# qiyunzhu/woltka

Hardware: AMD Instinct MI355X
Metric: alignment records/sec classified (higher is better)
Workload: dtype u8; 1 GPU; synthetic SAM text of 50M reads x <=16 hits (10.50 GB) resident in HBM, 2M-node taxonomy, ranks phylum,genus,species: device tokenizer per 64 MB block + one weighted histogram per sample (the kernels of `woltka classify`, host link left out); records_per_gpu=250034804, reads_per_gpu=50000000

## Files before the change

woltka_amd/csrc/wk_dtok_fused.hpp:

```cpp
#pragma once
#include "wk_dtok.hpp"
#include "wk_dtok_planes.hpp"

namespace wk {

constexpr uint32_t kFzThreads = 512;
constexpr uint32_t kFzWaves = kFzThreads / kWave;
constexpr uint32_t kFzTile = 16384;
constexpr uint32_t kFzBack = 1024;
constexpr uint32_t kFzFwd = 3072;
constexpr uint32_t kFzWin = kFzTile + kFzBack + kFzFwd;
constexpr uint32_t kFzChunks = kFzWin / 16 + 1;
constexpr uint32_t kFzChunksPerWave = (kFzChunks + kFzWaves - 1) / kFzWaves;
constexpr uint32_t kFzRounds = (kFzChunksPerWave + kWave - 1) / kWave;
constexpr uint32_t kFzLines = 1024;
constexpr uint32_t kFzStreams = 4;
constexpr uint32_t kFzCap = 1024;
static_assert(kFzCap >= kFzLines, "a window's records fit an empty buffer");
static_assert(kFzWin + 32 < 65536, "window offsets fit 16 bits");
constexpr uint32_t kFzCarry = 256;
static_assert(kFzCarry + kFzLines <= kFpMaxLines && kFzThreads % kWave == 0, "a window's owned lines fit the planes, a wave's lines one word");

constexpr uint32_t kDtokSpill = 64;

struct FusedArgs {
    const unsigned char* text;
    uint32_t n;
    uint32_t open_end;
    uint32_t span;
    const struct DictSlot8* dict8;
    const uint4* names16;
    uint32_t dict_mask;
    const unsigned char* arena;
    uint2* unknown;
    uint32_t unknown_cap;
    DtokState* state;
    DtokState* host_state;
    const unsigned long long* backup_prev;
    unsigned long long* backup_next;
    uint32_t* host_seq;
    uint32_t seq;
    StreamSet streams;
    const int32_t* submap;
    uint32_t n_submap;
    uint32_t ablate;
};

static_assert(sizeof(DtokState) % 8 == 0, "the packed totals are aligned");
__device__ __forceinline__ unsigned long long* fz_totals(DtokState* state) { return reinterpret_cast<unsigned long long*>(state + 1); }

__global__ void dtok_fused_begin_kernel(unsigned long long* __restrict__ backup, const unsigned long long* __restrict__ cursor, DtokState* state) {
    if (threadIdx.x < (uint32_t)kMaxStreams) backup[threadIdx.x] = cursor[threadIdx.x];
    if (threadIdx.x == 0) {
        *state = DtokState{0u, 0u, 0ull, 0ull, 0ull, 0u, 0u};
        *fz_totals(state) = 0ull;
    }
}

template <int kCtrl, int kRowMask>
__device__ __forceinline__ uint32_t fz_dpp_add(uint32_t v) {
    return v + (uint32_t)__builtin_amdgcn_update_dpp(0, (int)v, kCtrl, kRowMask, 0xF, false);
}
__device__ __forceinline__ uint32_t fz_wave_scan(uint32_t v) {
    static_assert(kWave == 64, "four rows of sixteen lanes");
    v = fz_dpp_add<0x111, 0xF>(v);
    v = fz_dpp_add<0x112, 0xF>(v);
    v = fz_dpp_add<0x114, 0xF>(v);
    v = fz_dpp_add<0x118, 0xF>(v);
    v = fz_dpp_add<0x142, 0xA>(v);
    v = fz_dpp_add<0x143, 0xC>(v);
    return v;
}
__device__ __forceinline__ uint32_t fz_last_lane(uint32_t v) { return (uint32_t)__builtin_amdgcn_readlane((int)v, kWave - 1); }
__device__ __forceinline__ uint32_t fz_wave_sum(uint32_t v) { return fz_last_lane(fz_wave_scan(v)); }
__device__ __forceinline__ unsigned long long fz_first_lane64(unsigned long long v) {
    return ((unsigned long long)(uint32_t)__builtin_amdgcn_readfirstlane((int)(uint32_t)(v >> 32)) << 32) |
           (uint32_t)__builtin_amdgcn_readfirstlane((int)(uint32_t)v);
}
constexpr uint32_t kFzNlBits = 11, kFzNlMask = (1u << kFzNlBits) - 1u;
static_assert(kFzRounds == 3 && kWave * 16u <= kFzNlMask, "two fields of 11 bits");
static_assert(kFzChunksPerWave > 2u * kWave && (kFzChunksPerWave - 2u * kWave) * 16u < (1u << (32u - 2u * kFzNlBits)), "and one of 10");

__device__ __forceinline__ uint4 fz_load_stream(const unsigned char* p) {
    typedef uint32_t u32x4 __attribute__((ext_vector_type(4)));
    const u32x4 v = __builtin_nontemporal_load(reinterpret_cast<const u32x4*>(p));
    return make_uint4(v.x, v.y, v.z, v.w);
}
__device__ __forceinline__ unsigned long long fz_load64(const unsigned char* p) {
    unsigned long long w;
    __builtin_memcpy(&w, p, 8);
    return w;
}
__device__ __forceinline__ uint32_t fz_load32(const unsigned char* p) {
    uint32_t w;
    __builtin_memcpy(&w, p, 4);
    return w;
}
__device__ __forceinline__ unsigned long long fz_eq_bytes(unsigned long long w, unsigned char c) {
    const unsigned long long x = w ^ (0x0101010101010101ull * c);
    return ~(((x & 0x7F7F7F7F7F7F7F7Full) + 0x7F7F7F7F7F7F7F7Full) | x | 0x7F7F7F7F7F7F7F7Full);
}
__device__ __forceinline__ uint32_t fz_marks32(uint32_t w, uint32_t c4) {
    const uint32_t x = w ^ c4;
    return ~(((x & 0x7F7F7F7Fu) + 0x7F7F7F7Fu) | x | 0x7F7F7F7Fu);
}
__device__ __forceinline__ unsigned long long fz_low_bytes(unsigned long long w, uint32_t k) {
    return k >= 8u ? w : (w & ((1ull << (8u * k)) - 1ull));
}

__device__ __forceinline__ unsigned long long fz_hash(const unsigned char* p, uint32_t n) {
    unsigned long long h = 0xcbf29ce484222325ull ^ ((unsigned long long)n * 0x9E3779B97F4A7C15ull);
    while (n >= 8u) {
        h = (h ^ fz_load64(p)) * 0x100000001b3ull;
        h ^= h >> 29;
        p += 8;
        n -= 8u;
    }
    const unsigned long long v = n ? fz_low_bytes(fz_load64(p), n) : 0ull;
    h = (h ^ v) * 0x100000001b3ull;
    h ^= h >> 32;
    h *= 0x9E3779B97F4A7C15ull;
    return h ^ (h >> 29);
}

__device__ __forceinline__ bool fz_same(const unsigned char* x, const unsigned char* y, uint32_t n) {
    while (n >= 8u) {
        if (fz_load64(x) != fz_load64(y)) return false;
        x += 8;
        y += 8;
        n -= 8u;
    }
    return n == 0u || fz_low_bytes(fz_load64(x) ^ fz_load64(y), n) == 0ull;
}

// ... 44 lines not shown
    while (pos > 0u) {
        const uint32_t e = pos - 1u;
        uint32_t s = e;
        while (s > 0u && text[s - 1u] != '\n') --s;
        uint32_t tab[3], nt = 0;
        for (uint32_t p = s; p < e && nt < 3u; ++p)
            if (text[p] == '\t') tab[nt++] = p;
        if (nt == 3u && !(tab[2] - tab[1] == 2u && text[tab[1] + 1u] == '*')) {
            if (tab[0] - s != qn) return true;
            for (uint32_t k = 0; k < qn; ++k)
                if (text[s + k] != q[k]) return true;
            return false;
        }
        pos = s;
    }
    return true;
}

constexpr uint32_t kFiSubj = (1u << 23) - 1u;
constexpr uint32_t kFiMateShift = 24;
constexpr uint32_t kFiMapped = 1u << 26;
constexpr uint32_t kFiStart = 1u << 27;
constexpr uint32_t kFiExcl = 1u << 29;
constexpr uint32_t kFiDropped = 1u << 30;
constexpr uint32_t kFiRead = kFiMapped | (3u << kFiMateShift);
constexpr uint32_t kFiKey = kFiRead | kFiSubj;
constexpr uint32_t kFzPad = 8;

__device__ __forceinline__ uint32_t fz_octet(uint32_t z_lo, uint32_t z_hi) { return (((z_lo >> 7) | (z_hi >> 3)) * 0x00204081u >> 21) & 255u; }

__device__ __forceinline__ uint32_t fz_newlines16(uint4 v) {
    return fz_octet(fz_marks32(v.x, 0x0A0A0A0Au), fz_marks32(v.y, 0x0A0A0A0Au)) | (fz_octet(fz_marks32(v.z, 0x0A0A0A0Au), fz_marks32(v.w, 0x0A0A0A0Au)) << 8);
}

__device__ __forceinline__ uint32_t fz_tabs32(const unsigned char* p) {
    unsigned long long w[4];
#pragma unroll
    for (uint32_t i = 0; i < 4; ++i) w[i] = fz_load64(p + 8u * i);
    uint32_t m = 0;
#pragma unroll
    for (uint32_t i = 0; i < 4; ++i)
        m |= fz_octet(fz_marks32((uint32_t)w[i], 0x09090909u), fz_marks32((uint32_t)(w[i] >> 32), 0x09090909u)) << (8u * i);
    return m;
}

__global__ void __launch_bounds__(kFzThreads) __attribute__((amdgpu_waves_per_eu(6, 6))) dtok_fused_kernel(FusedArgs a) {
    __shared__ __attribute__((aligned(16))) unsigned char txt[kFzChunks * 16 + 32];
    __shared__ uint16_t ls[kFzLines + 2];
    __shared__ uint16_t f_qn[kFzLines], f_rb[kFzLines], f_rn[kFzLines];
    __shared__ __attribute__((aligned(16))) uint32_t info_[kFzPad + kFzCarry + kFzLines + kFzPad + 8];
    __shared__ uint32_t carry[kFzCarry];
    __shared__ unsigned long long planes[kFpPlanes][kFpWords];
    __shared__ uint32_t rbuf[kFzStreams][kFzCap];
    __shared__ uint32_t rcnt[kFzStreams];
    __shared__ unsigned long long newc_packed;
    static_assert(kFzStreams <= 4 && kFzLines < 65536, "four 16-bit counts");
    __shared__ unsigned long long gbase[kFzStreams];
    __shared__ uint32_t wtot[kFzWaves];
    __shared__ unsigned long long gbase_out[kMaxStreams];
    __shared__ unsigned long long wg_totals;
    __shared__ uint32_t own[4];
    __shared__ uint32_t wg_flags;
    uint32_t* const info = info_ + kFzPad + kFzCarry;

    const uint32_t tid = threadIdx.x, lane = tid & (kWave - 1), wave = tid / kWave;
    const uint32_t n_streams = a.streams.n_streams;
    if (tid < kFzStreams) rcnt[tid] = 0u;
    if (tid == 0) newc_packed = 0ull;
    if (tid == 0) wg_flags = 0u;
    if (tid == 0) wg_totals = 0ull;
    uint32_t my_flags = 0, my_reads = 0, my_lines = 0;
    const uint32_t text_end = a.n + (a.open_end ? 1u : 0u);

    auto flush_all = [&](bool last) {
        __syncthreads();
        if (tid < n_streams) {
            const uint32_t cnt = (a.ablate & 64u) ? 0u : rcnt[tid];
            unsigned long long base = 0ull;
            if (cnt) {
                base = atomicAdd(&a.streams.cursor[tid], (unsigned long long)cnt);
                if (base + cnt > a.streams.cap) atomicOr(&wg_flags, kDtokSpill);
            }
            gbase[tid] = base;
        }
        __syncthreads();
        for (uint32_t k = 0; k < n_streams; ++k) {
            const uint32_t cnt = (a.ablate & 64u) ? 0u : rcnt[k];
            const unsigned long long base = gbase[k];
            for (uint32_t i = tid; i < cnt; i += kFzThreads)
                if (base + i < a.streams.cap) a.streams.out[k][base + i] = rbuf[k][i];
        }
        if (last) return;
        __syncthreads();
        if (tid < n_streams) rcnt[tid] = 0u;
        __syncthreads();
    };

    const uint32_t t0 = blockIdx.x * a.span;
    const uint32_t t1 = a.n - t0 > a.span ? t0 + a.span : a.n;
    const uint32_t span_w1 = (uint32_t)min((unsigned long long)t1 + kFzFwd, (unsigned long long)text_end);
    uint32_t wpos = t0 >= kFzBack ? t0 - kFzBack : 0u;
    uint32_t mode = 0u;
    uint32_t counted = t0;
    bool wide = false;
    uint32_t nc = 0u;
    uint32_t cq_pos = 0u, cq_len = 0u;
    const uint32_t max_trips = a.span / 16u + 2u;
    for (uint32_t trip = 0;; ++trip) {
        if (trip >= max_trips) {
            my_flags |= kDtokSpill;
            break;
        }
        const uint32_t w0 = wpos & ~15u;
        const uint32_t lead = wpos - w0;
        const uint32_t w1 = (uint32_t)min((mode == 0u ? (unsigned long long)t0 + kFzTile + kFzFwd : (unsigned long long)w0 + kFzWin),
                                           (unsigned long long)(wide ? text_end : span_w1));
        const bool to_end = w1 == text_end;
        const bool last_win = wide || w1 == span_w1;
        __syncthreads();
        if (tid < 3u) own[tid] = tid < 2u ? 0xFFFFFFFFu : 0u;
        if (tid < kFzPad) info[-(int32_t)nc - 1 - (int32_t)tid] = kFiStart;
        for (uint32_t i = tid; i < nc; i += kFzThreads) info[(int32_t)i - (int32_t)nc] = carry[i];

        uint4 v[kFzRounds];
#pragma unroll
        for (uint32_t r = 0; r < kFzRounds; ++r) {
            const uint32_t cw = r * kWave + lane;
            const uint32_t p = w0 + (wave * kFzChunksPerWave + cw) * 16u;
            v[r] = make_uint4(0u, 0u, 0u, 0u);
            if (cw < kFzChunksPerWave && p < a.n && p < w1) v[r] = fz_load_stream(a.text + p);
        }
        uint32_t marks[kFzRounds];
        uint32_t nl_packed = 0;
        const uint32_t in_lo = max(wpos, counted), in_hi = min(min(w1, a.n), t1);
        const uint32_t wave_c0 = (uint32_t)__builtin_amdgcn_readfirstlane((int)(wave * kFzChunksPerWave));
#pragma unroll
        for (uint32_t r = 0; r < kFzRounds; ++r) {
            const uint32_t cw = r * kWave + lane;
            const uint32_t c = wave * kFzChunksPerWave + cw;
            const uint32_t p = w0 + c * 16u;
            marks[r] = 0u;
            const uint32_t rc0 = wave_c0 + r * kWave, rp0 = w0 + rc0 * 16u;
            const bool interior = (r + 1u) * kWave <= kFzChunksPerWave && rc0 + kWave <= kFzChunks && rp0 >= in_lo &&
                                  (unsigned long long)rp0 + kWave * 16u <= in_hi;
            if (interior) {
                *reinterpret_cast<uint4*>(txt + c * 16u) = v[r];
                const uint32_t m = fz_newlines16(v[r]);
                const uint32_t cnt = (uint32_t)__popc(m);
                my_lines += cnt;
                marks[r] = m;
                nl_packed |= cnt << (kFzNlBits * r);
            } else if (cw < kFzChunksPerWave && c < kFzChunks) {
                *reinterpret_cast<uint4*>(txt + c * 16u) = v[r];
                if (p < w1) {
                    uint32_t m = fz_newlines16(v[r]);
                    if (p + 16u > a.n) m &= p >= a.n ? 0u : (1u << (a.n - p)) - 1u;
                    if (p >= counted && p < t1) my_lines += (uint32_t)__popc(m);
                    if (a.open_end && a.n >= p && a.n < p + 16u) m |= 1u << (a.n - p);
                    if (p + 16u > w1) m &= (1u << (w1 - p)) - 1u;
                    if (p < wpos) m &= ~((1u << (wpos - p)) - 1u);
                    marks[r] = m;
                    nl_packed |= (uint32_t)__popc(m) << (kFzNlBits * r);
                }
            }
        }
        const uint32_t nl_inc = fz_wave_scan(nl_packed);
        const uint32_t nl_wave = fz_last_lane(nl_inc);
        if (lane == 0) wtot[wave] = (nl_wave & kFzNlMask) + ((nl_wave >> kFzNlBits) & kFzNlMask) + (nl_wave >> (2u * kFzNlBits));
        __syncthreads();
        uint32_t before = 0, total_nl = 0;
#pragma unroll
        for (uint32_t w = 0; w < kFzWaves; ++w) {
            before += w < wave ? wtot[w] : 0u;
            total_nl += wtot[w];
        }
        const bool too_many = total_nl + 1u > kFzLines || (a.ablate & (32u | 512u));
        if (too_many) {
            if (!(a.ablate & 512u)) my_flags |= kDtokSpill;
        } else {
            if (tid == 0) ls[0] = (uint16_t)lead;
            uint32_t line = before;
#pragma unroll
            for (uint32_t r = 0; r < kFzRounds; ++r) {
                const uint32_t c = wave * kFzChunksPerWave + r * kWave + lane;
                uint32_t at = line + ((nl_inc >> (kFzNlBits * r)) & kFzNlMask) - (uint32_t)__popc(marks[r]);
                uint32_t m = marks[r];
                while (m) {
                    const uint32_t b = (uint32_t)__ffs((int)m) - 1u;
                    ls[++at] = (uint16_t)(c * 16u + b + 1u);
                    m &= m - 1u;
                }
                line += (nl_wave >> (kFzNlBits * r)) & kFzNlMask;
            }
        }
        __syncthreads();
        const uint32_t trail = too_many ? wpos : w0 + (uint32_t)__builtin_amdgcn_readfirstlane((int)(uint32_t)ls[total_nl]);
        if (!too_many && last_win && trail >= t0 && trail < t1) my_flags |= kDtokSpill;
        const uint32_t first_line = mode != 0u || w0 == 0u ? 0u : 1u;
        const uint32_t n_lines = too_many ? 0u : total_nl;
        if (tid == 0 && first_line) info[0] = 0u;

        for (uint32_t k = first_line + tid; k < n_lines; k += kFzThreads) {
            const uint32_t s = ls[k], e = (uint32_t)ls[k + 1] - 1u;
            uint32_t tab[3] = {0, 0, 0}, nt = 0;
            if (!(a.ablate & 256u)) {
                uint32_t m = fz_tabs32(txt + s);
                if (e - s < 32u) m &= (1u << (e - s)) - 1u;
                nt = min((uint32_t)__popc(m), 3u);
                tab[0] = s + (uint32_t)__ffs((int)m) - 1u;
                m &= m - 1u;
                tab[1] = s + (uint32_t)__ffs((int)m) - 1u;
                m &= m - 1u;
                tab[2] = s + (uint32_t)__ffs((int)m) - 1u;
                for (uint32_t p = s + 32u; nt < 3u && p < e; p += 32u) {
                    m = fz_tabs32(txt + p);
                    if (e - p < 32u) m &= (1u << (e - p)) - 1u;
                    for (; m && nt < 3u; m &= m - 1u) {
                        const uint32_t q = p + (uint32_t)__ffs((int)m) - 1u;
                        if (nt == 0u)
                            tab[0] = q;
                        else if (nt == 1u)
                            tab[1] = q;
                        else
                            tab[2] = q;
                        ++nt;
                    }
                }
            }
            uint32_t word = 0;
            if (a.ablate & 16u) {
            } else if (nt < 3u) {
                my_flags |= kDtokShortLine;
            } else {
                const uint32_t fl = tab[1] - tab[0] - 1u;
                const unsigned long long fw = fz_load64(txt + tab[0] + 1u);
                uint32_t flag = 0;
                bool digits = fl >= 1u && fl <= 6u;
                for (uint32_t i = 0; i < fl && i < 6u; ++i) {
                    const uint32_t d = ((uint32_t)(fw >> (8u * i)) & 0xFFu) - (uint32_t)'0';
                    digits &= d <= 9u;
                    flag = flag * 10u + d;
                }
                const uint32_t rb = tab[1] + 1u, rn = tab[2] - rb;
                if (!digits) {
                    my_flags |= kDtokShortLine;
                } else if (rn == 1u && txt[rb] == '*') {
                } else {
                    const uint32_t mate = (flag >> 6) & 3u;
                    if (mate == 3u) my_flags |= kDtokBothMates;
                    word = kFiMapped | (mate << kFiMateShift);
                    f_qn[k] = (uint16_t)(tab[0] - s);
                    f_rb[k] = (uint16_t)rb;
                    f_rn[k] = (uint16_t)rn;
                }
            }
            info[k] = word;
        }
        __syncthreads();

        for (uint32_t k = first_line + tid; k < n_lines; k += kFzThreads) {
            if (!(info[k] & kFiMapped) || w0 + ls[k] < t0) continue;
            const unsigned char* name = txt + f_rb[k];
            const uint32_t rn = f_rn[k];
            FzProbe probe;
            if (!(a.ablate & 1u)) probe = fz_probe_begin(a, name, rn);
            uint32_t j = k;
            bool found = false;
            while (j > first_line) {
                --j;
                if (info[j] & kFiMapped) {
                    found = true;
                    break;
                }
            }
            bool start;
            if (a.ablate & 8u)
                start = true;
            else if (found)
                start = f_qn[j] != f_qn[k] || !fz_same(txt + ls[k], txt + ls[j], f_qn[k]);
            else if (nc)
                start = f_qn[k] != cq_len || !fz_same(txt + ls[k], a.text + cq_pos, cq_len);
            else if (mode == 1u || wpos == 0u)
                start = true;
            else
                start = fz_starts_run_slow(a.text, w0 + ls[first_line], txt + ls[k], f_qn[k]);
            int32_t sid = (a.ablate & 1u) ? (int32_t)(fz_load32(name + 4) % 1000u) : fz_probe_end(a, probe, name, rn, w0 + f_rb[k]);
            bool excluded = false;
            if (a.submap && sid >= 0) {
                if ((uint32_t)sid < a.n_submap) {
                    sid = a.submap[sid];
                    if (sid == kLineExcluded) {
                        excluded = true;
                        sid = 0;
                    }
                } else {
                    my_flags |= kDtokSpill;
                    sid = -1;
                }
            }
            info[k] |= (start ? kFiStart : 0u) | (excluded ? kFiExcl : 0u) | (sid < 0 ? kFiSubj : ((uint32_t)sid & kFiSubj));
            if (start) {
                atomicMin(&own[w0 + ls[k] < t1 ? 0 : 1], k);
                atomicMax(&own[2], k);
            }
        }
        __syncthreads();
        const uint32_t o0 = (uint32_t)__builtin_amdgcn_readfirstlane((int)own[0]), o1 = (uint32_t)__builtin_amdgcn_readfirstlane((int)own[1]);
        const uint32_t last = (uint32_t)__builtin_amdgcn_readfirstlane((int)own[2]);
        const uint32_t lpos = w0 + (uint32_t)__builtin_amdgcn_readfirstlane((int)(uint32_t)ls[o0 != 0xFFFFFFFFu ? last : 0u]);
        const bool has_first = nc != 0u || o0 != 0xFFFFFFFFu;
        const int32_t first_own = nc ? -(int32_t)nc : (int32_t)o0;
        int32_t ka = 0, kb = 0;
        uint32_t next = 0u, next_mode = 0u, nc_next = 0u;
        bool more = false, again = false, put_aside = false;
        if (too_many) {
            if ((a.ablate & (32u | 512u)) && !last_win) {
                next = w1;
                next_mode = 2u;
                more = true;
            }
        } else if (o1 != 0xFFFFFFFFu) {
            kb = (int32_t)o1;
            ka = has_first ? first_own : kb;
        } else if (to_end) {
            kb = (int32_t)n_lines;
            ka = has_first ? first_own : kb;
        } else if (last_win && a.span <= kFzTile) {
            if (o0 != 0xFFFFFFFFu) my_flags |= kDtokSpill;
        } else if (o0 != 0xFFFFFFFFu && (nc != 0u || last != o0 || lpos > wpos)) {
            kb = (int32_t)last;
            ka = first_own;
            next = lpos;
            next_mode = 1u;
            more = true;
            again = last_win;
        } else if (o0 != 0xFFFFFFFFu && last_win && !wide) {
            next = wpos;
            next_mode = 1u;
            more = again = true;
        } else if (o0 != 0xFFFFFFFFu || nc != 0u) {
            put_aside = true;
        } else if (!last_win) {
            next = trail;
            next_mode = 2u;
            more = trail > wpos && trail < t1;
            if (trail <= wpos) my_flags |= kDtokSpill;
        }
        if (put_aside) {
            if (tid == 0) {
                uint32_t c = nc;
                for (uint32_t k = first_line; k < n_lines; ++k) {
                    const uint32_t w = info[k];
                    if (w & kFiMapped) {
                        if (c < kFzCarry) carry[c] = w & ~kFiDropped;
                        ++c;
                    }
                }
                own[3] = c;
            }
            __syncthreads();
            nc_next = (uint32_t)__builtin_amdgcn_readfirstlane((int)own[3]);
            if (nc_next > kFzCarry || trail <= wpos) {
                my_flags |= kDtokSpill;
                nc_next = 0u;
            } else {
                if (nc == 0u) {
                    cq_pos = wpos;
                    cq_len = (uint32_t)__builtin_amdgcn_readfirstlane((int)(uint32_t)f_qn[0]);
                }
                next = trail;
                next_mode = 2u;
                more = true;
                again = last_win;
            }
        }
        for (int32_t k0 = ka; k0 < kb; k0 += (int32_t)kFzThreads) {
            const int32_t k = k0 + (int32_t)tid;
            const uint32_t mk = k < kb ? info[k] : 0u;
            const bool mapped = (mk & kFiMapped) != 0u, excl = mapped && (mk & kFiExcl);
            if (excl) {
                int32_t j = k;
                while (!(info[j] & kFiStart)) --j;
                atomicOr(&info[j], kFiDropped);
            }
            bool dup = false;
            if (mapped && !excl && !(mk & kFiStart) && !(a.ablate & 2u)) {
                bool done = false;
                for (int32_t j = k; !done; j -= 8) {
                    uint32_t w[8];
#pragma unroll
                    for (uint32_t i = 0; i < 8; ++i) w[i] = info[j - 1 - (int32_t)i];
#pragma unroll
                    for (uint32_t i = 0; i < 8; ++i) {
                        dup |= !done && ((w[i] ^ mk) & kFiKey) == 0u;
                        done |= (w[i] & kFiStart) != 0u;
                    }
                }
            }
            const bool first = mapped && !excl && !dup;
            const uint32_t mate = (mk >> kFiMateShift) & 3u;
            const uint32_t wi = (uint32_t)__builtin_amdgcn_readfirstlane((int)((uint32_t)(k0 - ka) / kWave + wave));
            const bool put = lane == 0 && wi < kFpWords;
            const unsigned long long p_start = __ballot(mapped && (mk & kFiStart));
            if (put) planes[kFpStart][wi] = p_start;
#pragma unroll
            for (uint32_t m = 0; m < 4; ++m) {
                const unsigned long long p_first = __ballot(first && mate == m);
                if (put) planes[kFpFirst + m][wi] = p_first;
            }
        }
        __syncthreads();
        for (int32_t k0 = ka; k0 < kb; k0 += (int32_t)kFzThreads) {
            const int32_t k = k0 + (int32_t)tid;
            bool rec = false;
            uint32_t word = 0, sl = 0, at = 0;
            const uint32_t li = (uint32_t)(k - ka);
            const uint32_t mk = k < kb ? info[k] : 0u;
            const unsigned long long* const mine = planes[kFpFirst + ((mk >> kFiMateShift) & 3u)];
            if (k < kb && ((mine[li / 64u] >> (li % 64u)) & 1ull) && !(a.ablate & 4u)) {
                uint32_t pos = 0, size = 1;
                bool dropped = (mk & kFiStart) && (mk & kFiDropped);
                if (!(a.ablate & (2u | 128u))) {
                    const FpRead r = fp_read(planes[kFpStart], mine, li, (uint32_t)(kb - ka));
                    pos = r.pos;
                    size = r.size;
                    dropped = (info[ka + (int32_t)r.head] & kFiDropped) != 0u;
                }
                if (size > (uint32_t)WK_WEIGHT_MAX_K) my_flags |= kDtokBigRead;
                const uint32_t s = mk & kFiSubj;
                if (s != kFiSubj && !dropped) {
                    rec = true;
                    word = s | ((pos & 15u) << kWordSubjBits) | ((size & 31u) << kWordSizeShift);
                    sl = s / kSliceBins;
                    if (sl >= n_streams) sl = n_streams - 1u;
                    my_reads += pos == 0u ? 1u : 0u;
                }
            }
            {
                unsigned long long add = 0;
                uint32_t mine_before = 0;
                for (uint32_t s2 = 0; s2 < n_streams; ++s2) {
                    const unsigned long long m = __ballot(rec && sl == s2);
                    add |= (unsigned long long)__popcll(m) << (16u * s2);
                    if (rec && sl == s2) mine_before = (uint32_t)__popcll(m & ((1ull << lane) - 1ull));
                }
                if (add) {
                    unsigned long long base = 0;
                    if (lane == 0) base = atomicAdd(&newc_packed, add);
                    base = fz_first_lane64(base);
                    at = (uint32_t)(base >> (16u * sl)) & 0xFFFFu;
                    at += mine_before;
                }
            }
            __syncthreads();
            const unsigned long long newc = newc_packed;
            bool full = false;
            for (uint32_t s2 = 0; s2 < n_streams; ++s2) full |= rcnt[s2] + ((uint32_t)(newc >> (16u * s2)) & 0xFFFFu) > kFzCap;
            if (full) flush_all(false);
            if (rec) rbuf[sl][rcnt[sl] + at] = word;
            __syncthreads();
            if (tid < n_streams) rcnt[tid] += (uint32_t)(newc >> (16u * tid)) & 0xFFFFu;
            if (tid == 0) newc_packed = 0ull;
            __syncthreads();
        }
        if (!more) break;
        wpos = next;
        mode = next_mode;
        wide = again;
        nc = nc_next;
        counted = w1;
    }
    if (my_flags) atomicOr(&wg_flags, my_flags);
    {
        const uint32_t reads_w = fz_wave_sum(my_reads), lines_w = fz_wave_sum(my_lines);
        const unsigned long long t = ((unsigned long long)lines_w << 32) | reads_w;
        if (lane == 0 && t) atomicAdd(&wg_totals, t);
    }
    flush_all(true);
    __syncthreads();
    if (tid == 0) {
        if (wg_totals) __hip_atomic_fetch_add(fz_totals(a.state), wg_totals, __ATOMIC_RELAXED, __HIP_MEMORY_SCOPE_AGENT);
        if (wg_flags) atomicOr(&a.state->flags, wg_flags);
        __threadfence();
        own[0] = atomicAdd(&a.state->done, 1u) == gridDim.x - 1u ? 1u : 0u;
    }
    __syncthreads();
    if (own[0]) {
        __threadfence();
        if (tid < (uint32_t)kMaxStreams) {
            const unsigned long long cur = __hip_atomic_load(&a.streams.cursor[tid], __ATOMIC_RELAXED, __HIP_MEMORY_SCOPE_AGENT);
            a.backup_next[tid] = cur;
            gbase_out[tid] = tid < n_streams ? cur - a.backup_prev[tid] : 0ull;
        }
        __syncthreads();
        if (tid == 0) {
            DtokState st{};
            st.flags = __hip_atomic_load(&a.state->flags, __ATOMIC_RELAXED, __HIP_MEMORY_SCOPE_AGENT);
            st.n_unknown = __hip_atomic_load(&a.state->n_unknown, __ATOMIC_RELAXED, __HIP_MEMORY_SCOPE_AGENT);
            const unsigned long long totals = __hip_atomic_load(fz_totals(a.state), __ATOMIC_RELAXED, __HIP_MEMORY_SCOPE_AGENT);
            for (uint32_t k = 0; k < (uint32_t)kMaxStreams; ++k) st.n_out += gbase_out[k];
            st.n_reads = totals & 0xFFFFFFFFull;
            st.n_lines = totals >> 32;
            *a.host_state = st;
            *a.state = DtokState{0u, 0u, 0ull, 0ull, 0ull, 0u, 0u};
            *fz_totals(a.state) = 0ull;
            __threadfence_system();
            if (a.host_seq) __hip_atomic_store(a.host_seq, a.seq, __ATOMIC_RELEASE, __HIP_MEMORY_SCOPE_SYSTEM);
        }
    }
}

}
```

woltka_amd/csrc/woltka_hip.hip:

```cpp
#include <hip/hip_runtime.h>

#include <algorithm>
#include <atomic>
#include <ctime>
#include <chrono>
#include <cstdarg>
#include <cstdio>
#include <cstdlib>
#include <cstring>
#include <map>
#include <new>
#include <mutex>
#include <string>
#include <vector>

#include "../../include/woltka_hip.h"
#include "../../include/woltka_hip_measure.h"
#include "wk_classify.hpp"
#include "wk_cover.hpp"
#include "wk_device.hpp"
#include "wk_dtok.hpp"
#include "wk_dtok_fused.hpp"
#include "wk_free.hpp"
#include "wk_ordinal.hpp"
// ... 3146 lines not shown
                               c->d_tiles.as<unsigned long long>());
            hipLaunchKernelGGL(tile_scan_kernel, dim3(1), dim3(1024), 0, c->stream, c->d_tiles.as<unsigned long long>(),
                               c->d_tile_off.as<unsigned long long>(), (int64_t)n_tiles, scalar_u64(c, 3));
        }
        n_newlines = res->n_newlines;
        tile_off = res->tile_off;
        have_count = true;
    } else if (counted) {
        {
            Lap wait(&c->lap_s[3]);
            HIP_TRY(c, hipEventSynchronize(c->copy_ev[k]));
        }
        {
            float ms = 0.f;
            if (hipEventElapsedTime(&ms, c->copy_ev0[k], c->copy_evm[k]) == hipSuccess) {
                c->lap_copy_ms += ms;
                c->lap_copy_bytes += n;
            } else {
                (void)hipGetLastError();
            }
        }
        n_newlines = c->copy_newlines[k];
        tile_off = c->d_tile_off_k[k].as<unsigned long long>();
        have_count = true;
    } else if (want_count) {
        const int rc = count_now();
        if (rc) return rc;
    }
    const bool open_end = (ahead ? c->copy_last[k] : src[n - 1]) != '\n';
    uint32_t lines = (uint32_t)n_newlines + (open_end ? 1u : 0u);
    if (!have_count) {
        double est = (double)n / 7.0 + 1.0;
        if (c->dt_lpb > 0.0) est = std::min(est, (double)n * c->dt_lpb * 1.25 + 65536.0);
        lines = (uint32_t)est;
    }
    if (c->d_unknown.cap < (size_t)(1 << 20) * 8) HIP_TRY(c, c->d_unknown.reserve((size_t)(1 << 20) * 8));
    if (fuse) {
        c->dt_lines = lines;
        int rc = dtok_mirror_dict(c, tok);
        if (rc) return rc;
        if (c->dt_expect_bytes > 0 && c->w_expect == 0) {
            const double expect = (double)c->dt_expect_bytes * ((double)lines / (double)n) * 1.08 + (double)lines;
            c->w_expect = (int64_t)std::min(expect, (double)(1ll << 30));
        }
        if ((rc = words_roll(c, lines))) return rc;
        if ((rc = words_room(c, lines))) return rc;
        FusedArgs fa{};
        fa.streams = stream_set(c);
        if (c->w_mode == 0 && fa.streams.n_streams <= kFzStreams) {
            fa.text = c->dt_text;
            fa.n = n;
            fa.open_end = open_end ? 1u : 0u;
            const unsigned grid = fused_spans(c, n, &fa.span);
            fa.dict8 = c->d_dict2.as<DictSlot8>();
            fa.names16 = c->d_names16.as<uint4>();
            fa.dict_mask = c->dt_dict_mask;
            fa.arena = c->d_arena.as<unsigned char>();
            fa.unknown = c->d_unknown.as<uint2>();
            fa.unknown_cap = (uint32_t)(c->d_unknown.cap / 8);
            fa.state = c->d_state.as<DtokState>();
            fa.ablate = c->fused_ablate;
            fa.submap = c->dt_submap_on ? c->d_submap.as<int32_t>() : nullptr;
            fa.n_submap = c->dt_submap_n;
            c->w_counts_known = false;
            HIP_TRY(c, c->w_backup.reserve(kMaxStreams * 8));
            HIP_TRY(c, c->w_backup2.reserve(kMaxStreams * 8));
            HIP_TRY(c, c->w_backup3.reserve(kMaxStreams * 8));
            DevBuf& before = fz_bk(c, c->fz_parity);
            DevBuf& after = fz_bk(c, (c->fz_parity + 1) % 3);
            fa.backup_prev = before.as<unsigned long long>();
            fa.backup_next = after.as<unsigned long long>();
            fa.host_state = reinterpret_cast<DtokState*>(c->host_back);
            c->w_backup_cur = before.p;
            if (res) ktimer_end(c, kt);
            KernelTimer* kf = ktimer_begin(c, "dtok_fused");
            if (!c->fz_chain || c->fz_no_chain)
                hipLaunchKernelGGL(dtok_fused_begin_kernel, dim3(1), dim3(64), 0, c->stream, before.as<unsigned long long>(),
                                   (const unsigned long long*)fa.streams.cursor, fa.state);
            hipLaunchKernelGGL(dtok_fused_kernel, dim3(grid), dim3(kFzThreads), 0, c->stream, fa);
            ktimer_end(c, kf);
            HIP_TRY(c, hipGetLastError());
            lap_mark(2);
            DtokState st{};
            {
                Lap wait(&c->lap_s[2]);
                HIP_TRY(c, hipStreamSynchronize(c->stream));
            }
            small_back_get(c, 0, &st, sizeof st);
            lap_t = std::chrono::steady_clock::now();
            const bool keep = st.flags == 0 && st.n_unknown == 0;
            int64_t nr = 0, nrec = 0;
            c->dt_emitted = false;
            if ((rc = dtok_emit_finish(c, keep, false, st, 0, &nr, &nrec))) return rc;
            lap_mark(4);
            c->fused_streak = keep;
            c->fz_chain = keep;
            if (keep) {
                c->fz_parity = (c->fz_parity + 1) % 3;
                c->fz_back_streak = 0;
                ++c->fused_blocks;
                lines = (uint32_t)st.n_lines + (open_end ? 1u : 0u);
                c->dt_lines = lines;
                c->dt_lpb = (double)lines / (double)n;
                *status = 0;
                *n_lines = lines;
                *emit = 1;
// ... 141 lines not shown
    {
        std::lock_guard<std::mutex> lock(c->copy_mu);
        if (c->lag_count == 0)
            for (int q = 0; q < wk_ctx::kTextBufs; ++q)
                if (c->buf_state[q] == wk_ctx::kBufScanning) c->buf_state[q] = wk_ctx::kBufFree;
        if (!res) {
            for (int q = 0; q < wk_ctx::kTextBufs; ++q)
                if (c->buf_state[q] == wk_ctx::kBufCopied && c->copy_src[q] == src && c->copy_n[q] == n && (k < 0 || c->copy_seq[q] < c->copy_seq[k]))
                    k = q;
            if (k < 0) return WK_OK;
        }
    }
    if (res) {
        open_end = src[n - 1] != '\n';
        lines = (uint32_t)res->n_newlines + (open_end ? 1u : 0u);
    } else {
        if (c->dt_lpb <= 0.0) return WK_OK;
        open_end = c->copy_last[k] != '\n';
        lines = (uint32_t)std::min((double)n / 7.0 + 1.0, (double)n * c->dt_lpb * 1.25 + 65536.0);
    }
    int64_t under_way = lines;
    for (int i = 0; i < c->lag_count; ++i) under_way += c->lag[i].lines_est;
    if (c->w_records + under_way >= (1ll << 30) - (1 << 20)) return WK_OK;
    if (c->w_sliced && streams_needed(c) > kMaxStreams) return WK_OK;
    if (c->lag_count == 0) {
        const int rcw = words_room(c, under_way);
        if (rcw) return rcw;
    } else {
        const int want = c->w_sliced ? streams_needed(c) : 1;
        const size_t need = (size_t)(c->w_records + under_way) * 4 + 64;
        bool fits = c->w_cursor.p != nullptr && c->w_streams >= want;
        for (int q = 0; fits && q < c->w_streams; ++q) fits = need <= c->w_stream[q].cap;
        if (!fits) return WK_OK;
    }
    int rc = dtok_mirror_dict(c, tok);
    if (rc) return rc;
    FusedArgs fa{};
    fa.streams = stream_set(c);
    if (fa.streams.n_streams > kFzStreams) return WK_OK;
    if (!res) {
        std::lock_guard<std::mutex> lock(c->copy_mu);
        c->buf_state[k] = wk_ctx::kBufPending;
        c->copy_src[k] = nullptr;
        c->copy_counted[k] = false;
    }
    if (!res) HIP_TRY(c, hipStreamWaitEvent(c->stream, c->copy_ev[k], 0));
    HIP_TRY(c, c->d_state.reserve(sizeof(DtokState) + 64));
    if (c->d_unknown.cap < (size_t)(1 << 20) * 8) HIP_TRY(c, c->d_unknown.reserve((size_t)(1 << 20) * 8));
    for (int i = 0; i < 3; ++i) HIP_TRY(c, fz_bk(c, i).reserve(kMaxStreams * 8));
    fa.text = res ? res->dev : c->d_textptr[k];
    fa.n = n;
    fa.open_end = open_end ? 1u : 0u;
    const unsigned grid = fused_spans(c, n, &fa.span);
    fa.dict8 = c->d_dict2.as<DictSlot8>();
    fa.names16 = c->d_names16.as<uint4>();
    fa.dict_mask = c->dt_dict_mask;
    fa.arena = c->d_arena.as<unsigned char>();
    fa.unknown = c->d_unknown.as<uint2>();
    fa.unknown_cap = (uint32_t)(c->d_unknown.cap / 8);
    fa.state = c->d_state.as<DtokState>();
    fa.ablate = c->fused_ablate;
    fa.submap = c->dt_submap_on ? c->d_submap.as<int32_t>() : nullptr;
    fa.n_submap = c->dt_submap_n;
    wk_ctx::LagSlot& L = c->lag[c->lag_count];
    L.buf = res ? -1 : k;
    L.src = src;
    L.n = n;
    L.open_end = open_end;
    L.ring = c->fz_parity;
    L.lines_est = lines;
    L.host_slot = 2 + c->lag_next_ev;
    if (!c->lag_ev[c->lag_next_ev]) HIP_TRY(c, hipEventCreateWithFlags(&c->lag_ev[c->lag_next_ev], hipEventDisableTiming));
    L.ev = c->lag_ev[c->lag_next_ev];
    c->lag_next_ev ^= 1;
    fa.backup_prev = fz_bk(c, L.ring).as<unsigned long long>();
    fa.backup_next = fz_bk(c, (L.ring + 1) % 3).as<unsigned long long>();
    fa.host_state = reinterpret_cast<DtokState*>(c->host_back + (size_t)L.host_slot * wk_ctx::kBackBytes);
    static_assert(sizeof(DtokState) <= 128 && wk_ctx::kBackBytes >= 132, "the slot's second half holds the block's sequence number");
    L.seq = 0;
    if (c->lag_poll) {
        L.seq = ++c->lag_seq ? c->lag_seq : ++c->lag_seq;
        fa.host_seq = reinterpret_cast<uint32_t*>(c->host_back + (size_t)L.host_slot * wk_ctx::kBackBytes + 128);
        fa.seq = L.seq;
    }
    c->w_counts_known = false;
    KtScope kt_scope(c);
    KernelTimer* kf = ktimer_begin(c, "dtok_fused");
    if (!c->fz_chain || c->fz_no_chain)
        hipLaunchKernelGGL(dtok_fused_begin_kernel, dim3(1), dim3(64), 0, c->stream, fz_bk(c, L.ring).as<unsigned long long>(),
                           (const unsigned long long*)fa.streams.cursor, fa.state);
    hipLaunchKernelGGL(dtok_fused_kernel, dim3(grid), dim3(kFzThreads), 0, c->stream, fa);
    ktimer_end(c, kf);
    HIP_TRY(c, hipGetLastError());
    if (!c->lag_poll) HIP_TRY(c, hipEventRecord(L.ev, c->stream));
    c->fz_chain = true;
    c->fz_parity = (c->fz_parity + 1) % 3;
    ++c->lag_count;
    *started = 1;
    return WK_OK;
}

int wk_dtok_scan_emit_end(wk_ctx* c, int64_t* n_lines, int* status, int64_t* n_reads, int64_t* n_records) {
    if (!c || !n_lines || !status || !n_reads || !n_records) return WK_E_ARG;
    if (c->lag_count == 0) return fail(c, WK_E_STATE, "no block under way (wk_dtok_scan_emit_begin)");
    DeviceGuard guard(c->device);
    const wk_ctx::LagSlot L = c->lag[0];
// ... 1320 lines not shown
```

Before: 15.06 billion records/s.

## Deal window chunks unevenly across waves and drop per-batch record-count barriers

Splits the window's chunks so four waves take three rounds and four take two, replacing the padded per-wave share and narrowing the packed newline-count fields to 10 bits. Chunks with more than eight newlines are treated as malformed short lines. The per-stream record counts now live in a per-thread register copy of a packed atomic word, so the append step needs only one barrier per batch instead of three, and the last batch skips it. The full-buffer test becomes a single add-and-mask on the packed counts. In exchange it adds a requirement that spans be multiples of 16 bytes, and a new rejection path for dense newline chunks.

New measurement: 15.62 billion records/s, median of 6. 3.8% higher.

```diff
diff --git a/woltka_amd/csrc/wk_dtok_fused.hpp b/woltka_amd/csrc/wk_dtok_fused.hpp
--- a/woltka_amd/csrc/wk_dtok_fused.hpp
+++ b/woltka_amd/csrc/wk_dtok_fused.hpp
@@ -1,6 +1,7 @@
 #pragma once
 #include "wk_dtok.hpp"
 #include "wk_dtok_planes.hpp"
+#include "wk_dtok_rounds.hpp"
 
 namespace wk {
 
@@ -11,8 +12,9 @@
 constexpr uint32_t kFzFwd = 3072;
 constexpr uint32_t kFzWin = kFzTile + kFzBack + kFzFwd;
 constexpr uint32_t kFzChunks = kFzWin / 16 + 1;
-constexpr uint32_t kFzChunksPerWave = (kFzChunks + kFzWaves - 1) / kFzWaves;
-constexpr uint32_t kFzRounds = (kFzChunksPerWave + kWave - 1) / kWave;
+constexpr uint32_t kFzRounds = kFrMaxRounds;
+static_assert(kFrChunks * 16u == kFzWin && kFrTailChunk + 1u == kFzChunks && kFrWaves == kFzWaves && kFrWave == kWave,
+              "the dealing covers the window");
 constexpr uint32_t kFzLines = 1024;
 constexpr uint32_t kFzStreams = 4;
 constexpr uint32_t kFzCap = 1024;
@@ -77,9 +79,6 @@
     return ((unsigned long long)(uint32_t)__builtin_amdgcn_readfirstlane((int)(uint32_t)(v >> 32)) << 32) |
            (uint32_t)__builtin_amdgcn_readfirstlane((int)(uint32_t)v);
 }
-constexpr uint32_t kFzNlBits = 11, kFzNlMask = (1u << kFzNlBits) - 1u;
-static_assert(kFzRounds == 3 && kWave * 16u <= kFzNlMask, "two fields of 11 bits");
-static_assert(kFzChunksPerWave > 2u * kWave && (kFzChunksPerWave - 2u * kWave) * 16u < (1u << (32u - 2u * kFzNlBits)), "and one of 10");
 
 __device__ __forceinline__ uint4 fz_load_stream(const unsigned char* p) {
     typedef uint32_t u32x4 __attribute__((ext_vector_type(4)));
@@ -230,9 +229,8 @@
     __shared__ uint32_t carry[kFzCarry];
     __shared__ unsigned long long planes[kFpPlanes][kFpWords];
     __shared__ uint32_t rbuf[kFzStreams][kFzCap];
-    __shared__ uint32_t rcnt[kFzStreams];
-    __shared__ unsigned long long newc_packed;
-    static_assert(kFzStreams <= 4 && kFzLines < 65536, "four 16-bit counts");
+    __shared__ unsigned long long fill_packed;
+    static_assert(kFzStreams <= 4 && kFzCap + kFzThreads < 65536, "four 16-bit counts");
     __shared__ unsigned long long gbase[kFzStreams];
     __shared__ uint32_t wtot[kFzWaves];
     __shared__ unsigned long long gbase_out[kMaxStreams];
@@ -242,18 +240,22 @@
     uint32_t* const info = info_ + kFzPad + kFzCarry;
 
     const uint32_t tid = threadIdx.x, lane = tid & (kWave - 1), wave = tid / kWave;
+    const uint32_t wave_s = (uint32_t)__builtin_amdgcn_readfirstlane((int)wave);
     const uint32_t n_streams = a.streams.n_streams;
-    if (tid < kFzStreams) rcnt[tid] = 0u;
-    if (tid == 0) newc_packed = 0ull;
+    const uint32_t ablate = a.ablate;
+    const int32_t* const submap = a.submap;
+    unsigned long long fill = 0ull;
+    if (tid == 0) fill_packed = 0ull;
+    if (tid < 4u) reinterpret_cast<uint32_t*>(txt + kFrTailChunk * 16u)[tid] = 0u;
     if (tid == 0) wg_flags = 0u;
     if (tid == 0) wg_totals = 0ull;
     uint32_t my_flags = 0, my_reads = 0, my_lines = 0;
     const uint32_t text_end = a.n + (a.open_end ? 1u : 0u);
 
-    auto flush_all = [&](bool last) {
+    auto flush_all = [&](unsigned long long have, bool last) {
         __syncthreads();
         if (tid < n_streams) {
-            const uint32_t cnt = (a.ablate & 64u) ? 0u : rcnt[tid];
+            const uint32_t cnt = (ablate & 64u) ? 0u : (uint32_t)(have >> (16u * tid)) & 0xFFFFu;
             unsigned long long base = 0ull;
             if (cnt) {
                 base = atomicAdd(&a.streams.cursor[tid], (unsigned long long)cnt);
@@ -263,14 +265,12 @@
         }
         __syncthreads();
         for (uint32_t k = 0; k < n_streams; ++k) {
-            const uint32_t cnt = (a.ablate & 64u) ? 0u : rcnt[k];
+            const uint32_t cnt = (ablate & 64u) ? 0u : (uint32_t)(have >> (16u * k)) & 0xFFFFu;
             const unsigned long long base = gbase[k];
             for (uint32_t i = tid; i < cnt; i += kFzThreads)
                 if (base + i < a.streams.cap) a.streams.out[k][base + i] = rbuf[k][i];
         }
         if (last) return;
-        __syncthreads();
-        if (tid < n_streams) rcnt[tid] = 0u;
         __syncthreads();
     };
 
@@ -300,51 +300,49 @@
         if (tid < kFzPad) info[-(int32_t)nc - 1 - (int32_t)tid] = kFiStart;
         for (uint32_t i = tid; i < nc; i += kFzThreads) info[(int32_t)i - (int32_t)nc] = carry[i];
 
+        const uint32_t wave_c0 = fr_first_chunk(wave_s), wave_rounds = fr_rounds(wave_s);
         uint4 v[kFzRounds];
 #pragma unroll
         for (uint32_t r = 0; r < kFzRounds; ++r) {
-            const uint32_t cw = r * kWave + lane;
-            const uint32_t p = w0 + (wave * kFzChunksPerWave + cw) * 16u;
+            const uint32_t p = w0 + (wave_c0 + r * kWave + lane) * 16u;
             v[r] = make_uint4(0u, 0u, 0u, 0u);
-            if (cw < kFzChunksPerWave && p < a.n && p < w1) v[r] = fz_load_stream(a.text + p);
+            if (r < wave_rounds && p < a.n && p < w1) v[r] = fz_load_stream(a.text + p);
         }
         uint32_t marks[kFzRounds];
         uint32_t nl_packed = 0;
+        bool blank = false;
         const uint32_t in_lo = max(wpos, counted), in_hi = min(min(w1, a.n), t1);
-        const uint32_t wave_c0 = (uint32_t)__builtin_amdgcn_readfirstlane((int)(wave * kFzChunksPerWave));
 #pragma unroll
         for (uint32_t r = 0; r < kFzRounds; ++r) {
-            const uint32_t cw = r * kWave + lane;
-            const uint32_t c = wave * kFzChunksPerWave + cw;
+            const uint32_t c = wave_c0 + r * kWave + lane;
             const uint32_t p = w0 + c * 16u;
             marks[r] = 0u;
-            const uint32_t rc0 = wave_c0 + r * kWave, rp0 = w0 + rc0 * 16u;
-            const bool interior = (r + 1u) * kWave <= kFzChunksPerWave && rc0 + kWave <= kFzChunks && rp0 >= in_lo &&
-                                  (unsigned long long)rp0 + kWave * 16u <= in_hi;
+            if (r >= wave_rounds) continue;
+            const uint32_t rp0 = w0 + (wave_c0 + r * kWave) * 16u;
+            const bool interior = rp0 >= in_lo && (unsigned long long)rp0 + kWave * 16u <= in_hi;
+            *reinterpret_cast<uint4*>(txt + c * 16u) = v[r];
             if (interior) {
-                *reinterpret_cast<uint4*>(txt + c * 16u) = v[r];
-                const uint32_t m = fz_newlines16(v[r]);
+                const uint32_t m = fr_chunk_marks(fz_newlines16(v[r]), &blank);
                 const uint32_t cnt = (uint32_t)__popc(m);
                 my_lines += cnt;
                 marks[r] = m;
-                nl_packed |= cnt << (kFzNlBits * r);
-            } else if (cw < kFzChunksPerWave && c < kFzChunks) {
-                *reinterpret_cast<uint4*>(txt + c * 16u) = v[r];
-                if (p < w1) {
-                    uint32_t m = fz_newlines16(v[r]);
-                    if (p + 16u > a.n) m &= p >= a.n ? 0u : (1u << (a.n - p)) - 1u;
-                    if (p >= counted && p < t1) my_lines += (uint32_t)__popc(m);
-                    if (a.open_end && a.n >= p && a.n < p + 16u) m |= 1u << (a.n - p);
-                    if (p + 16u > w1) m &= (1u << (w1 - p)) - 1u;
-                    if (p < wpos) m &= ~((1u << (wpos - p)) - 1u);
-                    marks[r] = m;
-                    nl_packed |= (uint32_t)__popc(m) << (kFzNlBits * r);
-                }
-            }
-        }
+                nl_packed |= fr_pack(cnt, r);
+            } else if (p < w1) {
+                uint32_t m = fz_newlines16(v[r]);
+                if (p + 16u > a.n) m &= p >= a.n ? 0u : (1u << (a.n - p)) - 1u;
+                if (p >= counted && p < t1) my_lines += (uint32_t)__popc(m);
+                if (a.open_end && a.n >= p && a.n < p + 16u) m |= 1u << (a.n - p);
+                if (p + 16u > w1) m &= (1u << (w1 - p)) - 1u;
+                if (p < wpos) m &= ~((1u << (wpos - p)) - 1u);
+                m = fr_chunk_marks(m, &blank);
+                marks[r] = m;
+                nl_packed |= fr_pack((uint32_t)__popc(m), r);
+            }
+        }
+        if (blank && !(ablate & 16u)) my_flags |= kDtokShortLine;
         const uint32_t nl_inc = fz_wave_scan(nl_packed);
         const uint32_t nl_wave = fz_last_lane(nl_inc);
-        if (lane == 0) wtot[wave] = (nl_wave & kFzNlMask) + ((nl_wave >> kFzNlBits) & kFzNlMask) + (nl_wave >> (2u * kFzNlBits));
+        if (lane == 0) wtot[wave] = fr_total(nl_wave);
         __syncthreads();
         uint32_t before = 0, total_nl = 0;
 #pragma unroll
@@ -352,23 +350,24 @@
             before += w < wave ? wtot[w] : 0u;
             total_nl += wtot[w];
         }
-        const bool too_many = total_nl + 1u > kFzLines || (a.ablate & (32u | 512u));
+        const bool too_many = total_nl + 1u > kFzLines || (ablate & (32u | 512u));
         if (too_many) {
-            if (!(a.ablate & 512u)) my_flags |= kDtokSpill;
+            if (!(ablate & 512u)) my_flags |= kDtokSpill;
         } else {
             if (tid == 0) ls[0] = (uint16_t)lead;
             uint32_t line = before;
 #pragma unroll
             for (uint32_t r = 0; r < kFzRounds; ++r) {
-                const uint32_t c = wave * kFzChunksPerWave + r * kWave + lane;
-                uint32_t at = line + ((nl_inc >> (kFzNlBits * r)) & kFzNlMask) - (uint32_t)__popc(marks[r]);
+                if (r >= wave_rounds) continue;
+                const uint32_t c = wave_c0 + r * kWave + lane;
+                uint32_t at = line + fr_unpack(nl_inc, r) - (uint32_t)__popc(marks[r]);
                 uint32_t m = marks[r];
                 while (m) {
                     const uint32_t b = (uint32_t)__ffs((int)m) - 1u;
                     ls[++at] = (uint16_t)(c * 16u + b + 1u);
                     m &= m - 1u;
                 }
-                line += (nl_wave >> (kFzNlBits * r)) & kFzNlMask;
+                line += fr_unpack(nl_wave, r);
             }
         }
         __syncthreads();
@@ -381,7 +380,7 @@
         for (uint32_t k = first_line + tid; k < n_lines; k += kFzThreads) {
             const uint32_t s = ls[k], e = (uint32_t)ls[k + 1] - 1u;
             uint32_t tab[3] = {0, 0, 0}, nt = 0;
-            if (!(a.ablate & 256u)) {
+            if (!(ablate & 256u)) {
                 uint32_t m = fz_tabs32(txt + s);
                 if (e - s < 32u) m &= (1u << (e - s)) - 1u;
                 nt = min((uint32_t)__popc(m), 3u);
@@ -406,7 +405,7 @@
                 }
             }
             uint32_t word = 0;
-            if (a.ablate & 16u) {
+            if (ablate & 16u) {
             } else if (nt < 3u) {
                 my_flags |= kDtokShortLine;
             } else {
@@ -441,7 +440,7 @@
             const unsigned char* name = txt + f_rb[k];
             const uint32_t rn = f_rn[k];
             FzProbe probe;
-            if (!(a.ablate & 1u)) probe = fz_probe_begin(a, name, rn);
+            if (!(ablate & 1u)) probe = fz_probe_begin(a, name, rn);
             uint32_t j = k;
             bool found = false;
             while (j > first_line) {
@@ -452,7 +451,7 @@
                 }
             }
             bool start;
-            if (a.ablate & 8u)
+            if (ablate & 8u)
                 start = true;
             else if (found)
                 start = f_qn[j] != f_qn[k] || !fz_same(txt + ls[k], txt + ls[j], f_qn[k]);
@@ -462,11 +461,11 @@
                 start = true;
             else
                 start = fz_starts_run_slow(a.text, w0 + ls[first_line], txt + ls[k], f_qn[k]);
-            int32_t sid = (a.ablate & 1u) ? (int32_t)(fz_load32(name + 4) % 1000u) : fz_probe_end(a, probe, name, rn, w0 + f_rb[k]);
+            int32_t sid = (ablate & 1u) ? (int32_t)(fz_load32(name + 4) % 1000u) : fz_probe_end(a, probe, name, rn, w0 + f_rb[k]);
             bool excluded = false;
-            if (a.submap && sid >= 0) {
+            if (submap && sid >= 0) {
                 if ((uint32_t)sid < a.n_submap) {
-                    sid = a.submap[sid];
+                    sid = submap[sid];
                     if (sid == kLineExcluded) {
                         excluded = true;
                         sid = 0;
@@ -492,7 +491,7 @@
         uint32_t next = 0u, next_mode = 0u, nc_next = 0u;
         bool more = false, again = false, put_aside = false;
         if (too_many) {
-            if ((a.ablate & (32u | 512u)) && !last_win) {
+            if ((ablate & (32u | 512u)) && !last_win) {
                 next = w1;
                 next_mode = 2u;
                 more = true;
@@ -562,7 +561,7 @@
                 atomicOr(&info[j], kFiDropped);
             }
             bool dup = false;
-            if (mapped && !excl && !(mk & kFiStart) && !(a.ablate & 2u)) {
+            if (mapped && !excl && !(mk & kFiStart) && !(ablate & 2u)) {
                 bool done = false;
                 for (int32_t j = k; !done; j -= 8) {
                     uint32_t w[8];
@@ -595,10 +594,10 @@
             const uint32_t li = (uint32_t)(k - ka);
             const uint32_t mk = k < kb ? info[k] : 0u;
             const unsigned long long* const mine = planes[kFpFirst + ((mk >> kFiMateShift) & 3u)];
-            if (k < kb && ((mine[li / 64u] >> (li % 64u)) & 1ull) && !(a.ablate & 4u)) {
+            if (k < kb && ((mine[li / 64u] >> (li % 64u)) & 1ull) && !(ablate & 4u)) {
                 uint32_t pos = 0, size = 1;
                 bool dropped = (mk & kFiStart) && (mk & kFiDropped);
-                if (!(a.ablate & (2u | 128u))) {
+                if (!(ablate & (2u | 128u))) {
                     const FpRead r = fp_read(planes[kFpStart], mine, li, (uint32_t)(kb - ka));
                     pos = r.pos;
                     size = r.size;
@@ -624,22 +623,24 @@
                 }
                 if (add) {
                     unsigned long long base = 0;
-                    if (lane == 0) base = atomicAdd(&newc_packed, add);
+                    if (lane == 0) base = atomicAdd(&fill_packed, add);
                     base = fz_first_lane64(base);
                     at = (uint32_t)(base >> (16u * sl)) & 0xFFFFu;
                     at += mine_before;
                 }
             }
             __syncthreads();
-            const unsigned long long newc = newc_packed;
-            bool full = false;
-            for (uint32_t s2 = 0; s2 < n_streams; ++s2) full |= rcnt[s2] + ((uint32_t)(newc >> (16u * s2)) & 0xFFFFu) > kFzCap;
-            if (full) flush_all(false);
-            if (rec) rbuf[sl][rcnt[sl] + at] = word;
-            __syncthreads();
-            if (tid < n_streams) rcnt[tid] += (uint32_t)(newc >> (16u * tid)) & 0xFFFFu;
-            if (tid == 0) newc_packed = 0ull;
-            __syncthreads();
+            unsigned long long now = fz_first_lane64(fill_packed);
+            static_assert(kFzCap + 0x7BFFu == 0x7FFFu && 2u * kFzCap + kFzThreads + 0x7BFFu < 0x10000u, "the full test");
+            if ((now + 0x7BFF7BFF7BFF7BFFull) & 0x8000800080008000ull) {
+                flush_all(fill, false);
+                at -= (uint32_t)(fill >> (16u * sl)) & 0xFFFFu;
+                now -= fill;
+                if (tid == 0) fill_packed = now;
+            }
+            if (rec) rbuf[sl][at] = word;
+            fill = now;
+            if (k0 + (int32_t)kFzThreads < kb) __syncthreads();
         }
         if (!more) break;
         wpos = next;
@@ -654,7 +655,7 @@
         const unsigned long long t = ((unsigned long long)lines_w << 32) | reads_w;
         if (lane == 0 && t) atomicAdd(&wg_totals, t);
     }
-    flush_all(true);
+    flush_all(fill, true);
     __syncthreads();
     if (tid == 0) {
         if (wg_totals) __hip_atomic_fetch_add(fz_totals(a.state), wg_totals, __ATOMIC_RELAXED, __HIP_MEMORY_SCOPE_AGENT);
@@ -665,10 +666,12 @@
     __syncthreads();
     if (own[0]) {
         __threadfence();
-        if (tid < (uint32_t)kMaxStreams) {
-            const unsigned long long cur = __hip_atomic_load(&a.streams.cursor[tid], __ATOMIC_RELAXED, __HIP_MEMORY_SCOPE_AGENT);
-            a.backup_next[tid] = cur;
-            gbase_out[tid] = tid < n_streams ? cur - a.backup_prev[tid] : 0ull;
+        uint32_t xt = tid;
+        asm volatile("" : "+v"(xt));
+        if (xt < (uint32_t)kMaxStreams) {
+            const unsigned long long cur = __hip_atomic_load(&a.streams.cursor[xt], __ATOMIC_RELAXED, __HIP_MEMORY_SCOPE_AGENT);
+            a.backup_next[xt] = cur;
+            gbase_out[xt] = xt < n_streams ? cur - a.backup_prev[xt] : 0ull;
         }
         __syncthreads();
         if (tid == 0) {
diff --git a/woltka_amd/csrc/wk_dtok_rounds.hpp b/woltka_amd/csrc/wk_dtok_rounds.hpp
--- /dev/null
+++ b/woltka_amd/csrc/wk_dtok_rounds.hpp
@@ -0,0 +1,41 @@
+#pragma once
+#include <cstdint>
+
+#if defined(__HIPCC__) || defined(__CUDACC__)
+#define WK_FR_FN __host__ __device__ __forceinline__
+#else
+#define WK_FR_FN inline
+#endif
+
+namespace wk {
+
+constexpr uint32_t kFrWave = 64;
+constexpr uint32_t kFrWaves = 8;
+constexpr uint32_t kFrLongWaves = 4;
+constexpr uint32_t kFrMaxRounds = 3;
+constexpr uint32_t kFrChunks = (kFrLongWaves * 3u + (kFrWaves - kFrLongWaves) * 2u) * kFrWave;
+constexpr uint32_t kFrTailChunk = kFrChunks;
+constexpr uint32_t kFrChunkMax = 8;
+constexpr uint32_t kFrNlBits = 10, kFrNlMask = (1u << kFrNlBits) - 1u;
+static_assert(kFrChunkMax * kFrWave <= kFrNlMask, "a round's running sum fits its field");
+static_assert(kFrMaxRounds * kFrNlBits <= 32u, "three fields in a word");
+
+WK_FR_FN uint32_t fr_rounds(uint32_t w) { return w < kFrLongWaves ? 3u : 2u; }
+WK_FR_FN uint32_t fr_chunks(uint32_t w) { return fr_rounds(w) * kFrWave; }
+WK_FR_FN uint32_t fr_first_chunk(uint32_t w) {
+    return w < kFrLongWaves ? w * 3u * kFrWave : kFrLongWaves * 3u * kFrWave + (w - kFrLongWaves) * 2u * kFrWave;
+}
+
+WK_FR_FN uint32_t fr_chunk_marks(uint32_t marks16, bool* blank) {
+    if ((uint32_t)__builtin_popcount(marks16) > kFrChunkMax) {
+        *blank = true;
+        return 0u;
+    }
+    return marks16;
+}
+
+WK_FR_FN uint32_t fr_pack(uint32_t count, uint32_t round) { return count << (kFrNlBits * round); }
+WK_FR_FN uint32_t fr_unpack(uint32_t word, uint32_t round) { return (word >> (kFrNlBits * round)) & kFrNlMask; }
+WK_FR_FN uint32_t fr_total(uint32_t word) { return fr_unpack(word, 0) + fr_unpack(word, 1) + fr_unpack(word, 2); }
+
+}
diff --git a/woltka_amd/csrc/woltka_hip.hip b/woltka_amd/csrc/woltka_hip.hip
--- a/woltka_amd/csrc/woltka_hip.hip
+++ b/woltka_amd/csrc/woltka_hip.hip
@@ -3222,6 +3222,7 @@
             fa.n = n;
             fa.open_end = open_end ? 1u : 0u;
             const unsigned grid = fused_spans(c, n, &fa.span);
+            if (fa.span % 16u) return fail(c, WK_E_ARG, "spans of the one-kernel tokenizer are multiples of 16 bytes");
             fa.dict8 = c->d_dict2.as<DictSlot8>();
             fa.names16 = c->d_names16.as<uint4>();
             fa.dict_mask = c->dt_dict_mask;
@@ -3469,6 +3470,7 @@
     fa.n = n;
     fa.open_end = open_end ? 1u : 0u;
     const unsigned grid = fused_spans(c, n, &fa.span);
+    if (fa.span % 16u) return fail(c, WK_E_ARG, "spans of the one-kernel tokenizer are multiples of 16 bytes");
     fa.dict8 = c->d_dict2.as<DictSlot8>();
     fa.names16 = c->d_names16.as<uint4>();
     fa.dict_mask = c->dt_dict_mask;
```
